# wolfbox/snappy

Hardware: AMD Instinct MI355X
Metric: GiB/s hashed (whole node), bit-exact hashes.yaml, 10k x 1 MiB tree (higher is better)
Workload: dtype u64; 1 GPU; C2: ONE on-disk tree (tmpfs) of 10001 files (10 000 x 1 MiB + the 1 MiB archive stand-in) -> hashes.yaml, sharded over 1 rank(s) on 1 distinct GPU(s); bytes=10486808576, kernel=sha512_split_kernel<true>, tree_home=/dev/shm

## Files before the change

snappy_amd/csrc/hostpass.cpp:

```cpp
#include "hostpass.h"

#include "hostfill.h"
#include "walk.h"

#include <dirent.h>
#include <errno.h>
#include <string.h>
#include <sys/stat.h>

#include <algorithm>
#include <string_view>
#include <functional>
#include <queue>
#include <thread>

namespace snaphash {


int mode_string(uint32_t st_mode, char out[11])
{
    memcpy(out, "----------", 11);
    if (S_ISDIR(st_mode)) out[0] = 'd';
    else if (S_ISLNK(st_mode)) out[0] = 'l';
    else if (S_ISREG(st_mode)) out[0] = 'f';
// ... 2 lines not shown
    for (int i = 0; i < 9; ++i)
        if (st_mode & (1u << (8 - i))) out[i + 1] = rwx[i];
    return SNAPHASH_OK;
}

int mode_parse(const char* s, uint32_t* st_mode)
{
    if (!s || !s[0]) return SNAPHASH_EPARSE;
    uint32_t m;
    switch (s[0]) {
    case 'd': m = S_IFDIR; break;
    case 'f': m = S_IFREG; break;
    case 'l': m = S_IFLNK; break;
    default: return SNAPHASH_EPARSE;
    }
    static const char rwx[] = "rwxrwxrwx";
    for (int i = 0; i < 9 && s[i + 1]; ++i)
        if (s[i + 1] == rwx[i]) m |= 1u << (8 - i);
    *st_mode = m;
    return SNAPHASH_OK;
}


static int records_from_entries_impl(std::vector<WalkEntry>& ents, std::vector<Record>& out, bool steal)
{
    if (ents.empty()) return SNAPHASH_OK;
    const size_t rootlen = ents[0].path.size();
    const size_t n = ents.size();
    const unsigned T = (unsigned)std::max<size_t>(1, std::min<size_t>(std::min(8u, usable_cpus()), n / 2048));
    std::vector<uint8_t> keep(n, 0);
    std::vector<size_t> kept(T + 1, 0), bad(T, n);
    auto range = [&](unsigned t, size_t& lo, size_t& hi) { lo = n * t / T; hi = n * (t + 1) / T; };
    run_on_threads(T, [&](unsigned t) {
        size_t lo, hi, c = 0;
        range(t, lo, hi);
        for (size_t i = lo; i < hi; ++i) {
            const char* rel = ents[i].path.c_str() + rootlen;
            if (rel[0] == 0 || strncmp(rel, "/DEBIAN", 7) == 0) continue;
            char m[11];
            if (mode_string(ents[i].st.st_mode, m) != SNAPHASH_OK) { bad[t] = i; break; }
            keep[i] = 1;
            ++c;
        }
        kept[t + 1] = c;
    });
    size_t first_bad = n;
    for (unsigned t = 0; t < T; ++t) first_bad = std::min(first_bad, bad[t]);
    if (first_bad < n) return SNAPHASH_EMODE;
    for (unsigned t = 0; t < T; ++t) kept[t + 1] += kept[t];
    const size_t base = out.size();
    out.resize(base + kept[T]);
    run_on_threads(T, [&](unsigned t) {
        size_t lo, hi;
        range(t, lo, hi);
        size_t at = base + kept[t];
        for (size_t i = lo; i < hi; ++i) {
            if (!keep[i]) continue;
            WalkEntry& e = ents[i];
            Record& r = out[at++];
            r.name.assign(e.path.c_str() + rootlen + 1, e.path.size() - rootlen - 1);
            r.st_mode = e.st.st_mode;
            r.is_regular = S_ISREG(e.st.st_mode);
            r.size = r.is_regular ? (int64_t)e.st.st_size : 0;
            if (steal) r.path = std::move(e.path);
            else r.path = e.path;
        }
    });
    return SNAPHASH_OK;
}

size_t first_unemittable_name(const std::vector<Record>& recs)
{
    const size_t n = recs.size();
    const unsigned T = (unsigned)std::max<size_t>(1, std::min<size_t>(std::min(8u, usable_cpus()), n / 2048));
    std::vector<size_t> bad(T, n);
    run_on_threads(T, [&](unsigned t) {
        for (size_t i = n * t / T; i < n * (t + 1) / T; ++i)
            if (!name_emittable(recs[i].name)) { bad[t] = i; break; }
    });
    size_t first = n;
    for (size_t b : bad) first = std::min(first, b);
    return first;
}

int records_from_entries(const std::vector<WalkEntry>& ents, std::vector<Record>& out)
{
    return records_from_entries_impl(const_cast<std::vector<WalkEntry>&>(ents), out, false);
}

int walk_tree(const char* build_dir, std::vector<Record>& out, int* err_no)
{
    std::vector<WalkEntry> ents;
    int e = 0;
    const int wrc = walk_entries(build_dir, ents, &e, nullptr);
    if (err_no) *err_no = e;
    const int rc = records_from_entries_impl(ents, out, true);
    if (rc) return rc;
    return wrc ? SNAPHASH_EIO : SNAPHASH_OK;
}


bool plain_safe_name(const std::string& s)
{
    if (s.empty() || s.size() > 72) return false;
    bool alpha = false;
    for (unsigned char c : s) {
        const bool ok = (c >= 'a' && c <= 'z') || (c >= 'A' && c <= 'Z') || (c >= '0' && c <= '9') || c == '_' ||
                        c == '.' || c == '/' || c == '-' || c == '+';
        if (!ok) return false;
        if ((c >= 'a' && c <= 'z') || (c >= 'A' && c <= 'Z')) alpha = true;
    }
    const unsigned char c0 = s[0];
    if (c0 == '-' || c0 == '.' || c0 == '+' || (c0 >= '0' && c0 <= '9')) return false;
    if (!alpha) return false;
    static const char* const resolved[] = {"y", "Y", "yes", "Yes", "YES", "on", "On", "ON", "n", "N", "no", "No", "NO",
                                           "off", "Off", "OFF", "true", "True", "TRUE", "false", "False", "FALSE",
                                           "null", "Null", "NULL", nullptr};
    if (s.size() <= 5)
        for (int i = 0; resolved[i]; ++i)
// ... 562 lines not shown
```

snappy_amd/csrc/hostpass.h:

```cpp
#pragma once
#include <stdint.h>
#include <stdio.h>

#include <string>
#include <vector>

#include "../../include/snaphash.h"

namespace snaphash {

struct Record {
    std::string name;
    std::string path;
    uint32_t st_mode = 0;
    bool is_regular = false;
    int64_t size = 0;
    std::string sha512_hex;
};

struct ParsedRecord {
    std::string name, sha512_hex;
    int64_t size = 0;
    uint32_t st_mode = 0;
    bool has_name = false, has_size = false, has_mode = false;
};
struct ParsedHashes {
    bool has_archive = false;
    std::string archive_hex;
    std::vector<ParsedRecord> files;
};

int mode_string(uint32_t st_mode, char out[11]);
int mode_parse(const char* s, uint32_t* st_mode);
int walk_tree(const char* build_dir, std::vector<Record>& out, int* err_no);
struct WalkEntry;
int records_from_entries(const std::vector<WalkEntry>& ents, std::vector<Record>& out);
bool plain_safe_name(const std::string& s);
int yaml_append_name_scalar(const std::string& s, int column, int indent, std::string& out);
bool name_emittable(const std::string& s);
size_t first_unemittable_name(const std::vector<Record>& recs);
void hex_lower(const uint8_t d[64], char out[128]);
int emit_yaml(const std::vector<Record>& recs, const uint8_t archive_digest[64], const uint8_t* file_digests,
              std::string& out);
struct YamlSkeleton {
    std::string text;
    std::vector<size_t> hex_at;
};
int emit_yaml_skeleton(const std::vector<Record>& recs, YamlSkeleton& out, unsigned max_threads = 8 );
void yaml_fill_digests(YamlSkeleton& sk, const uint8_t archive_digest[64], const uint8_t* file_digests);
int shard_listing(const char* build_dir, uint32_t rank, uint32_t world, std::string& blob, int* err_no);
int records_from_listings(const char* build_dir, uint32_t world, const void* const* blobs, const size_t* blob_lens, std::vector<Record>& recs);
int parse_yaml(const char* text, size_t len, ParsedHashes& out);
bool digest_matches_hex(const uint8_t d[64], const std::string& hex);
int lpt_assign(const uint64_t* lens, size_t n, int nshards, int32_t* shard_of);

}
```

snappy_amd/csrc/snaphash_api.cpp:

```cpp
#include <dirent.h>
#include <errno.h>
#include <fcntl.h>
#include <hip/hip_runtime.h>
#include <string.h>
#include <sys/resource.h>
#include <sys/stat.h>
#include <unistd.h>

#include <algorithm>
#include <atomic>
#include <queue>
#include <chrono>
#include <string>
#include <thread>
#include <unordered_map>
#include <vector>

#include <dlfcn.h>
#include <rccl/rccl.h>

#include <condition_variable>
#include <functional>
#include <future>
#include <memory>
#include <mutex>

#include "engine_bufs.h"
#include "hostfill.h"
#include "hostpass.h"
#include "hostsha.h"
#include "inflate_host.h"
#include "member_hashers.h"
#include "planner.h"
#include "sha512_core.h"
#include "sha512_kernels.h"
// ... 371 lines not shown
    const unsigned T = (unsigned)std::min<size_t>(cap, std::max<size_t>(1, ops.size() / 4));
    const double t_fill0 = now_ms();
    struct FillAccount {
        DevCtx* c; const std::vector<ReadOp>& ops; unsigned T; double t0;
        ~FillAccount()
        {
            uint64_t b = 0;
            for (const ReadOp& op : ops) b += op.n;
            c->fill_bytes += b;
            c->fill_thread_s += (now_ms() - t0) * 1e-3 * T;
        }
    } account{c, ops, T, t_fill0};
    c->pool.parallel_for(ops.size(), T, [&](size_t i) {
        if (first_err.load(std::memory_order_relaxed)) return;
        const ReadOp& op = ops[i];
        const int err = do_read_op(src[op.src], op, cache);
        if (err) {
            int z = 0;
            if (first_err.compare_exchange_strong(z, err)) first_err_src.store(op.src);
        }
    });
}

int hash_sources(DevCtx* c, const std::vector<Source>& src, uint8_t* digests, uint64_t* states, int* err_no,
                 int64_t* err_src)
{
    const size_t n = src.size();
    if (err_no) *err_no = 0;
    if (err_src) *err_src = -1;
    if (n == 0) return SNAPHASH_OK;
    HIP_TRY(c, hipSetDevice(c->device));
    uint64_t job_bytes = 0;
    for (const Source& sc : src) job_bytes += sc.gpu_len;
    const unsigned nslots = job_bytes > 2 * c->staging ? 3u : 2u;
    uint64_t slot_bytes = std::min<uint64_t>(c->staging, 8u << 20);
    while (slot_bytes < c->staging && slot_bytes < job_bytes / 2 + kAlign * n) slot_bytes <<= 1;
    slot_bytes = std::min(slot_bytes, c->staging);
    for (unsigned k = 0; k < nslots; ++k) slot_bytes = std::max(slot_bytes, std::min(c->slot[k].cap(), c->staging));
    int rc = ensure_slots(c, (int)nslots, slot_bytes);
    if (rc) return rc;
    HIP_TRY(c, c->hash.ensure(n, true));

    c->fill_thread_s = 0;
    c->fill_bytes = 0;
    std::vector<uint64_t> done(n, 0);
    std::vector<uint32_t> active;
    active.reserve(n);
    for (size_t i = 0; i < n; ++i)
        if (src[i].gpu_len > 0 || src[i].len == 0) active.push_back((uint32_t)i);
    std::stable_sort(active.begin(), active.end(), [&](uint32_t a, uint32_t b) { return src[a].gpu_len > src[b].gpu_len; });
    std::atomic<int> first_err{0};
    std::atomic<int64_t> first_err_src{-1};
    std::vector<ReadOp> ops;
    const bool from_memory = src[0].mem != nullptr;
    FdCache fds(from_memory ? 0 : n, c->fd_call_budget >= 0 ? std::min(c->fd_call_budget, c->fd_budget) : c->fd_budget);
    const uint64_t seg_floor = from_memory ? kMinSegmentMem : kMinSegment;
    uint64_t S_full = slot_bytes;
    if (job_bytes + kAlign * n > slot_bytes && (slot_bytes & (slot_bytes - 1)) == 0 && slot_bytes > (32u << 20)) {
        S_full = 32u << 20;
        while (S_full < slot_bytes && (S_full < job_bytes / 24 || S_full < (seg_floor + kAlign) * std::min<uint64_t>(n, kTargetStreams))) S_full <<= 1;
    }
    const unsigned per_slot = (unsigned)(slot_bytes / S_full), nsub = nslots * per_slot;
    if (c->sub.size() < nsub) c->sub.resize(nsub);
    for (unsigned q = 0; q < nsub; ++q) {
        SubSlot& ss = c->sub[q];
        if (!ss.done) HIP_TRY(c, hipEventCreateWithFlags(&ss.done, hipEventDisableTiming));
        if (!ss.copied) HIP_TRY(c, hipEventCreateWithFlags(&ss.copied, hipEventDisableTiming));
        ss.busy = false;
    }
    const size_t n_active0 = active.size();
    const size_t new_cap = [] {
        const char* e = getenv("SNAPHASH_NEW_PER_BATCH");
        return e ? (size_t)strtoul(e, nullptr, 10) : (size_t)1024;
    }();
    const bool hold_back_on = [] { const char* e = getenv("SNAPHASH_HOLD_BACK"); return !e || atoi(e) != 0; }();
    bool held_back = false;
    const unsigned ramp_shift = [] {
        const char* e = getenv("SNAPHASH_RAMP_SHIFT");
        const unsigned long v = e ? strtoul(e, nullptr, 10) : 3ul;
        return (unsigned)std::min<unsigned long>(std::max<unsigned long>(v, 1), 8);
    }();
    unsigned ramp_first64 = 24, ramp_growth_pct = 115;
    if (const char* e = getenv("SNAPHASH_RAMP_MANY")) {
        unsigned a = 0, b = 0;
        if (sscanf(e, "%u,%u", &a, &b) == 2 && a >= 1 && a <= 64 && b >= 100 && b <= 400) { ramp_first64 = a; ramp_growth_pct = b; }
    }
    unsigned batch = 0;
    double t_wait = 0, t_plan = 0, t_read = 0, t_launch = 0;
    const double t_engine0 = now_ms();
    double t_first_copy = 0;
    size_t n_copies = 0;

    while (!active.empty()) {
        const unsigned q = batch % nsub;
        SubSlot& sl = c->sub[q];
        uint8_t* const sl_h = c->slot[q / per_slot].h_buf.data() + (uint64_t)(q % per_slot) * S_full;
        uint8_t* const sl_d = c->slot[q / per_slot].d_buf.data() + (uint64_t)(q % per_slot) * S_full;
        const double tb0 = now_ms();
        if (sl.busy) { HIP_TRY(c, hipEventSynchronize(sl.done)); sl.busy = false; }
        const double tb1 = now_ms();
        t_wait += tb1 - tb0;
        long double total_rem = 0;
        size_t n_started = 0;
        for (uint32_t id : active) { total_rem += (long double)(src[id].gpu_len - done[id]); n_started += done[id] != 0; }
        uint64_t S = S_full;
        if (job_bytes + kAlign * n > S_full) {
            if (n_active0 > 2048 && ramp_growth_pct > 100) {
                double f = (double)ramp_first64 / 64.0;
                for (unsigned k = 0; k < batch && f < 1.0; ++k) f *= (double)ramp_growth_pct / 100.0;
                if (f < 1.0) S = std::max<uint64_t>((uint64_t)((double)S_full * f) & ~(uint64_t)(kAlign - 1), std::min<uint64_t>(S_full, 1u << 20));
            } else if (batch < ramp_shift) {
                const uint64_t every = active.size() <= 2048 ? std::min<uint64_t>(S_full, (seg_floor + kAlign) * (uint64_t)active.size()) : 0;
                S = std::max<uint64_t>({(S_full >> (ramp_shift - batch)) & ~(uint64_t)(kAlign - 1), every & ~(uint64_t)(kAlign - 1), std::min<uint64_t>(S_full, 1u << 20)});
            }
            if (total_rem < 2 * (long double)S) {
                const uint64_t half = ((uint64_t)(total_rem / 2) + kAlign * active.size()) & ~(uint64_t)(kAlign - 1);
                const uint64_t least = std::max<uint64_t>(S_full >> 5, (seg_floor + kAlign) * active.size());
                if (half >= least) S = std::min(S, half);
            }
        }
        const bool cap_new = new_cap != 0 && !from_memory && n_active0 > 2048;
        const size_t n_serve = cap_new ? std::min<size_t>(kTargetStreams, n_started + std::min<size_t>(new_cap, active.size() - n_started)) : kTargetStreams;
        const uint64_t floor_q = std::max<uint64_t>(seg_floor, (S / std::max<size_t>(1, n_serve)) & ~(uint64_t)(kAlign - 1));
        const uint64_t pad = kAlign * (uint64_t)active.size();
        const uint64_t S_share = pad < S / 2 ? S - pad : S;
        HIP_TRY(c, sl.jobs.ensure(active.size()));

        ops.clear();
        size_t nj = 0;
        uint64_t used = 0;
        std::vector<uint32_t> still, skipped, floor_still;
        still.reserve(active.size());
        constexpr uint64_t kHold = 16u << 10;
        const bool hold_back = hold_back_on && !held_back && n_active0 > 2048 && total_rem <= (long double)S_share && total_rem > (long double)(8u << 20) &&
                               total_rem > (long double)(kHold + kHold / 2) * (long double)active.size();
        if (hold_back) held_back = true;
        bool full = false;
        size_t n_new = 0;
        const bool share_all = total_rem > (long double)S;
        const long double share_ratio = share_all ? (long double)S_share / total_rem : 1.0L;
        for (size_t ai = 0; ai < active.size(); ++ai) {
            const uint32_t id = active[ai];
            if (full) { skipped.insert(skipped.end(), active.begin() + (ptrdiff_t)ai, active.end()); break; }
            if (cap_new && done[id] == 0 && src[id].gpu_len != 0) {
                if (n_new >= new_cap) { skipped.push_back(id); continue; }
                ++n_new;
            }
            const uint64_t rem = src[id].gpu_len - done[id];
            uint64_t quota = share_all ? (uint64_t)((long double)rem * share_ratio) : rem;
            const bool at_floor = (quota & ~(uint64_t)(kAlign - 1)) < floor_q;
            quota = std::max(quota & ~(uint64_t)(kAlign - 1), floor_q);
            uint64_t take = rem <= quota ? rem : quota;
            if (hold_back) {
                if (rem <= kHold + kHold / 2) { skipped.push_back(id); continue; }
                take = std::min<uint64_t>(take, (rem - kHold) & ~(uint64_t)(kAlign - 1));
            }
            const uint64_t at = (used + kAlign - 1) & ~(uint64_t)(kAlign - 1);
            if (at + take > S) { full = true; skipped.push_back(id); continue; }
            const bool last = take == rem;
            const bool fin = last && src[id].gpu_len == src[id].len;
            Job j;
            j.data = (uint64_t)(uintptr_t)(sl_d + at);
            j.nbytes = take;
            j.total_prev = done[id];
            j.idx = id;
            j.flags = (done[id] == 0 ? kJobFirst : 0u) | (fin ? kJobFinal : 0u);
            sl.jobs.h[nj++] = j;
            if (take) ops.push_back(ReadOp{id, done[id], take, sl_h + at, fin && src[id].path != nullptr});
            used = at + take;
            done[id] += take;
            c->stats.blocks += padded_blocks(take, fin);
            if (!last) (at_floor ? floor_still : still).push_back(id);
        }
        still.insert(still.end(), skipped.begin(), skipped.end());
        still.insert(still.end(), floor_still.begin(), floor_still.end());
        active.swap(still);
        static const bool trace_batches = getenv("SNAPHASH_TRACE_BATCHES") != nullptr;
        if (trace_batches) {
            uint64_t mx = 0;
            for (size_t k = 0; k < nj; ++k) mx = std::max<uint64_t>(mx, sl.jobs.h[k].nbytes);
            fprintf(stderr, "snaphash engine %d: batch %u: S %llu, %zu segments, %llu bytes, largest share %llu, %zu streams left behind\n", c->index, batch,
                    (unsigned long long)S, nj, (unsigned long long)used, (unsigned long long)mx, active.size());
        }
        const double tb2 = now_ms();
        t_plan += tb2 - tb1;

        run_reads(c, src, ops, first_err, first_err_src, from_memory ? nullptr : &fds, batch == 0);
        if (first_err.load()) break;
        const double tb3 = now_ms();
        t_read += tb3 - tb2;
        if (trace_batches)
            fprintf(stderr, "snaphash engine %d: batch %u: at %.2f ms: waited %.2f, planned %.2f, filled %.2f ms (%zu streams begun, %.1f GB/s)\n", c->index, batch,
                    tb0 - t_engine0, tb1 - tb0, tb2 - tb1, tb3 - tb2, n_new, (double)used / ((tb3 - tb2) * 1e6 + 1e-9));
// ... 18 lines not shown
    const double ts0 = now_ms();
    static const bool trace_tree = getenv("SNAPHASH_TRACE_TREE") != nullptr;
    float gpu_span = 0, copy_busy = 0, copy_span = 0;
    if (trace_tree && c->ev_used > 1) {
        if (c->copy_stream) (void)hipStreamSynchronize(c->copy_stream);
        (void)hipStreamSynchronize(c->stream);
        size_t first_copy = c->ev_used, last_copy = 0, last_kernel = 0;
        for (size_t i = 0; i < c->ev_used; ++i) {
            float ms = 0;
            if (c->ev_pool[i].kind == 1) {
                if (first_copy == c->ev_used) first_copy = i;
                last_copy = i;
                if (hipEventElapsedTime(&ms, c->ev_pool[i].a, c->ev_pool[i].b) == hipSuccess) copy_busy += ms;
            } else if (c->ev_pool[i].kind == 0) last_kernel = i;
        }
        if (first_copy < c->ev_used) {
            (void)hipEventElapsedTime(&gpu_span, c->ev_pool[first_copy].a, c->ev_pool[last_kernel].b);
            (void)hipEventElapsedTime(&copy_span, c->ev_pool[first_copy].a, c->ev_pool[last_copy].b);
        }
    }
    rc = sync_ctx(c);
    if (trace_tree)
        fprintf(stderr, "snaphash engine %d: %u batches; waiting for a slot %.1f ms, planning %.1f ms, reads %.1f ms, enqueue %.1f ms, drain %.1f ms; "
                        "first copy enqueued at %.2f ms, copies busy %.2f of %.2f ms, first copy -> last kernel %.2f ms, engine %.2f ms\n",
                c->index, batch, t_wait, t_plan, t_read, t_launch, now_ms() - ts0, t_first_copy, copy_busy, copy_span, gpu_span, now_ms() - t_engine0);
    for (SubSlot& ss : c->sub) ss.busy = false;
    if (rc) return rc;
    if (first_err.load()) {
        const int64_t s = first_err_src.load();
        if (err_no) *err_no = first_err.load();
        if (err_src) *err_src = s;
        return fail(c, SNAPHASH_EIO,
                    std::string(s >= 0 && src[s].path ? src[s].path : "<buffer>") + ": " + strerror(first_err.load()));
    }
    if (digests) HIP_TRY(c, hipMemcpy(digests, c->hash.d_digests.data(), n * 64, hipMemcpyDeviceToHost));
    if (states) HIP_TRY(c, hipMemcpy(states, c->hash.d_state.data(), n * 64, hipMemcpyDeviceToHost));
    for (size_t i = 0; i < n; ++i) c->stats.bytes_hashed += src[i].gpu_len;
    c->stats.streams = n;
    if (c->owner) {
        std::lock_guard<std::mutex> lk(c->owner->calib_mu);
        const double planned = c->owner->ex.planned_gpu_ms, took = now_ms() - t_engine0;
        const bool take_fill = c->staged_calls++ > 0 && !(planned > 0 && took > 3.0 * planned);
        c->owner->calib.observe_call(!from_memory, (double)c->fill_bytes, (double)n, (double)n_copies, c->stats.h2d_ms * 1e-3, c->fill_thread_s, take_fill);
    }
    return SNAPHASH_OK;
}


bool rccl_load(snaphash_ctx* x)
{
    Rccl& r = x->rccl;
    if (r.tried) return r.ok;
    r.tried = true;
    for (const char* name : {"librccl.so.1", "librccl.so", "/opt/rocm/lib/librccl.so.1"}) {
        r.lib = dlopen(name, RTLD_NOW | RTLD_LOCAL);
        if (r.lib) break;
    }
    if (!r.lib) { r.why = "librccl.so not found"; return false; }
    r.CommInitAll = (decltype(r.CommInitAll))dlsym(r.lib, "ncclCommInitAll");
    r.CommDestroy = (decltype(r.CommDestroy))dlsym(r.lib, "ncclCommDestroy");
    r.AllGather = (decltype(r.AllGather))dlsym(r.lib, "ncclAllGather");
    r.GroupStart = (decltype(r.GroupStart))dlsym(r.lib, "ncclGroupStart");
    r.GroupEnd = (decltype(r.GroupEnd))dlsym(r.lib, "ncclGroupEnd");
    r.GetErrorString = (decltype(r.GetErrorString))dlsym(r.lib, "ncclGetErrorString");
    if (!r.CommInitAll || !r.CommDestroy || !r.AllGather || !r.GroupStart || !r.GroupEnd) {
        r.why = "librccl.so lacks a required symbol";
// ... 148 lines not shown
        t.bytes_hashed += s.bytes_hashed;
        t.blocks += s.blocks;
        t.streams += s.streams;
        t.launches += s.launches;
        if (s.launches) t.kernel_used = s.kernel_used;
        t.kernel_ms = std::max(t.kernel_ms, s.kernel_ms);
        t.h2d_ms = std::max(t.h2d_ms, s.h2d_ms);
    }
    x->ex.gpu_bytes = t.bytes_hashed;
    t.bytes_hashed += x->ex.host_bytes;
    t.streams += x->ex.host_streams;
    t.wall_ms = x->stats.wall_ms;
    x->stats = t;
}

void begin_top(snaphash_ctx* x)
{
    x->stats = snaphash_stats{};
    x->ex = snaphash_stats_ex{};
    x->ex.struct_size = sizeof(snaphash_stats_ex);
    x->ex.n_devices = (uint32_t)x->dev.size();
    x->last_error.clear();
    for (auto& d : x->dev) { begin_call(d.get()); d->t_call0 = 0; }
}

bool keep_on_device_planned(const snaphash_ctx* x, size_t nd) { return nd > 1 || (x->flags & SNAPHASH_FLAG_FORCE_GATHER); }

int hash_sources_top(snaphash_ctx* x, std::vector<Source>& src, uint8_t* digests, int32_t* status)
{
    const size_t n = src.size();
    if (status) for (size_t i = 0; i < n; ++i) status[i] = 0;
    if (n == 0) return SNAPHASH_OK;
    const size_t nd = x->dev.size();
    for (Source& s : src) s.gpu_len = s.len;
    std::vector<uint8_t> on_host(n, 0);
    unsigned plan_threads = 0;
    const double t_hash0 = now_ms();
    struct HashClock {
        snaphash_ctx* x; double t0;
        ~HashClock() { x->ex.hash_ms = now_ms() - t0; }
    } hash_clock{x, t_hash0};
    if (!x->gpu_only) {
        std::vector<uint64_t> lens(n);
        for (size_t i = 0; i < n; ++i) lens[i] = src[i].len;
        PlanResult plan = plan_streams(lens.data(), n, plan_model_of(x, src[0].path != nullptr));
        on_host.swap(plan.on_host);
// ... 37 lines not shown
        DevJob& J = job[d];
        J.sub.reserve(member[d].size());
        for (uint32_t g : member[d]) J.sub.push_back(src[g]);
        if (!keep_on_device) J.dig.resize(J.sub.size() * 64);
        J.rc = hash_sources(x->dev[d].get(), J.sub, keep_on_device ? nullptr : J.dig.data(), nullptr, &J.err_no, &J.err_src);
    };

    std::atomic<size_t> hnext{0};
    std::atomic<int> herr{0};
    std::atomic<int64_t> herr_src{-1};
    unsigned nh = hidx.empty() ? 0u : std::max(1u, std::min<unsigned>(plan_threads, (unsigned)hidx.size()));
    const bool gpu_part = !gidx.empty();
    const bool spare_cores = 2u * nh <= (x->cpus_call ? x->cpus_call : x->cpus);
    std::vector<double> hbusy(std::max(1u, nh), 0.0);
    std::stable_sort(hidx.begin(), hidx.end(), [&](uint32_t a, uint32_t b) { return src[a].len > src[b].len; });
    uint64_t host_bytes_planned = 0;
    for (uint32_t g : hidx) host_bytes_planned += src[g].len;
    const uint64_t alone_from = nh ? host_bytes_planned / nh / 4 : 0;
    size_t n_lane_streams = 0;
    for (uint32_t g : hidx) n_lane_streams += src[g].len < alone_from || alone_from == 0;
    unsigned host_lanes = nh ? (unsigned)std::min<size_t>(8, (n_lane_streams + nh - 1) / nh) : 1u;
    for (auto& d : x->dev) d->fd_call_budget = -1;
    if (src[0].path != nullptr) {
        struct rlimit rl;
        int64_t soft = 1024;
        if (getrlimit(RLIMIT_NOFILE, &rl) == 0) soft = rl.rlim_cur == RLIM_INFINITY ? 65536 : (int64_t)rl.rlim_cur;
        const int64_t held = soft < 8192 ? open_descriptors() + 16 : 0;
        const int64_t reserve = std::max<int64_t>(held, std::min<int64_t>(512, soft / 2));
        const int64_t transient = gpu_part ? (int64_t)std::min(x->d0()->fill_cap, 12u) * (int64_t)nd : 0;
        const int64_t pool = std::max<int64_t>(2, soft - reserve - transient);
        int64_t lanes_fds = (int64_t)nh * host_lanes;
        const int64_t lanes_cap = gpu_part ? std::max<int64_t>(1, pool / 2) : pool;
        if (lanes_fds > lanes_cap) {
            if ((int64_t)nh > lanes_cap) nh = (unsigned)lanes_cap;
            host_lanes = (unsigned)std::max<int64_t>(1, lanes_cap / nh);
            lanes_fds = (int64_t)nh * host_lanes;
        }
        for (auto& d : x->dev) d->fd_call_budget = std::max<int64_t>(0, (pool - lanes_fds) / (int64_t)nd);
    }
    auto run_host = [&](unsigned t) {
        const double t0 = now_ms();
        int64_t bad = -1;
        const int err = host_sha512_many(
            host_lanes,
            [&]() -> int64_t {
                if (herr.load()) return -1;
                const size_t k = hnext.fetch_add(1);
                return k < hidx.size() ? (int64_t)hidx[k] : -1;
            },
            [&](int64_t g) {
                HostStream h;
                h.mem = src[g].mem;
                h.path = src[g].mem ? nullptr : src[g].path;
// ... 118 lines not shown
        ThreadJoiner th;
        for (unsigned t = 1; t < T; ++t) th.spawn(work, t);
        work(0);
        th.join_all();
        int64_t first = -1;
        for (unsigned t = 0; t < T; ++t) if (bad[t] >= 0 && (first < 0 || bad[t] < first)) first = bad[t];
        if (first >= 0) {
            int err = EIO;
            int64_t b = first_bad_path(paths, (size_t)first + 1, &err);
            if (b < 0) b = first;
            if (status) { for (size_t k = 0; k < n; ++k) status[k] = 0; status[b] = err; }
            return fail(x, SNAPHASH_EIO, std::string(paths[b]) + ": " + strerror(err));
        }
    }
    const int rc = hash_sources_top(x, src, digests, status);
    if (rc == SNAPHASH_EIO) {
        int err = 0;
        const int64_t bad = first_bad_path(paths, n, &err);
        if (bad >= 0) {
            if (status) { for (size_t k = 0; k < n; ++k) status[k] = 0; status[bad] = err; }
            return fail(x, SNAPHASH_EIO, std::string(paths[bad]) + ": " + strerror(err));
        }
    }
    return rc;
}

void end_top(snaphash_ctx* x, double t0) { x->stats.wall_ms = now_ms() - t0; }

}


extern "C" {

int snaphash_abi_version(void) { return SNAPHASH_ABI_VERSION; }

static thread_local std::string g_init_error;

static int init_fail(int code, const std::string& what, hipError_t e = hipSuccess)
try {
    g_init_error = what + (e != hipSuccess ? std::string(": ") + hipGetErrorString(e) : std::string());
    return code;
} catch (...) {
    return SNAPHASH_ENOMEM;
}

static void destroy_dev(DevCtx* c)
// ... 284 lines not shown
    c->stats.streams = n;
    return lift(x, c, launch_jobs(c, c->hash.jobs.h.data(), c->hash.jobs.d.data(), n, (uint8_t*)d_digests));
} catch (...) {
    return SNAPHASH_ENOMEM;
}

int snaphash_sync(snaphash_ctx* x)
try {
    if (!x) return SNAPHASH_EINVAL;
    for (auto& d : x->dev) {
        HIP_TRY(d.get(), hipSetDevice(d->device));
        int rc = sync_ctx(d.get());
        if (rc) return lift(x, d.get(), rc);
    }
    const double wall = x->d0()->stats.wall_ms;
    merge_stats(x);
    if (x->stats.wall_ms == 0) x->stats.wall_ms = wall;
    return SNAPHASH_OK;
} catch (...) {
    return SNAPHASH_ENOMEM;
}


static int tree_impl(snaphash_ctx* x, const char* build_dir, const char* data_tar, const uint8_t* archive_digest,
                     std::string& yaml)
{
    struct stat st;
    if (data_tar && stat(data_tar, &st) != 0) return fail(x, SNAPHASH_EIO, std::string(data_tar) + ": " + strerror(errno));
    std::vector<Record> recs;
    int en = 0;
    const double tw0 = now_ms();
    int rc = walk_tree(build_dir, recs, &en);
    const double tw1 = now_ms();
    if (rc) return fail(x, rc, rc == SNAPHASH_EIO ? std::string(build_dir) + ": " + strerror(en) : "Unknown file mode");
    if (const size_t b = first_unemittable_name(recs); b < recs.size())
        return fail(x, SNAPHASH_ENAME, "name outside what the YAML emitter restates (yamlscalar.cpp): " + recs[b].name);
    std::vector<const char*> paths;
    std::vector<int64_t> sizes;
    if (data_tar) { paths.push_back(data_tar); sizes.push_back(-1); }
    for (const Record& r : recs)
        if (r.is_regular) { paths.push_back(r.path.c_str()); sizes.push_back(r.size); }
    std::vector<uint8_t> dig(paths.size() * 64 + 64);
    const double th0 = now_ms();
    const bool early_yaml = recs.size() >= 2048;
    YamlSkeleton sk;
    int sk_rc = SNAPHASH_OK;
    ThreadJoiner skt;
    if (early_yaml) skt.spawn([&recs, &sk, &sk_rc] { sk_rc = emit_yaml_skeleton(recs, sk, 1); });
    rc = hash_paths(x, paths.data(), paths.size(), sizes.data(), dig.data(), nullptr);
    skt.join_all();
    const double th1 = now_ms();
// ... 1338 lines not shown
```

snappy_amd/csrc/walk.cpp:

```cpp
#include "walk.h"

#include "hostfill.h"

#include <dirent.h>
#include <errno.h>
#include <fcntl.h>
#include <string.h>

#include <stdio.h>
#include <stdlib.h>

#include <algorithm>
#include <atomic>
#include <chrono>
#include <thread>

namespace snaphash {

namespace {

struct Child {
    std::string name;
    unsigned char type = DT_UNKNOWN;
    struct stat st;
// ... 59 lines not shown
        const unsigned T = walk_threads(hi - lo, 4);
        std::atomic<size_t> next{lo};
        run_on_threads(T, [&](unsigned) {
            for (;;) {
                const size_t i = next.fetch_add(1);
                if (i >= hi) return;
                list_dir(dirs[i]);
            }
        });
        for (size_t i = lo; i < hi; ++i)
            for (size_t k = 0; k < dirs[i].kids.size(); ++k)
                if (dirs[i].kids[k].type == DT_DIR && !dirs[i].kids[k].lstat_errno) {
                    dirs[i].kids[k].dir = (int64_t)dirs.size();
                    DirList sub;
                    sub.path = dirs[i].path + "/" + dirs[i].kids[k].name;
                    dirs.push_back(std::move(sub));
                }
        lo = hi;
    }
}

}

int walk_entries(const char* root_c, std::vector<WalkEntry>& ents, int* err_no, std::string* err_path)
{
    std::string root(root_c);
    while (root.size() > 1 && root.back() == '/') root.pop_back();
    if (err_no) *err_no = 0;
    ents.clear();
    ents.resize(1);
    ents[0].path = root;
    if (lstat(root.c_str(), &ents[0].st) != 0) {
        if (err_no) *err_no = errno;
        if (err_path) *err_path = root;
        ents.clear();
        return -1;
    }
    ents[0].have_st = true;
    if (!S_ISDIR(ents[0].st.st_mode)) return 0;
    const bool trace = getenv("SNAPHASH_TRACE_TREE") != nullptr;
    const auto t0 = std::chrono::steady_clock::now();
    std::vector<DirList> dirs;
    list_tree(root, dirs);
    const auto t1 = std::chrono::steady_clock::now();

    const size_t nd = dirs.size();
    std::vector<size_t> count(nd, 0), start(nd, 0);
    for (size_t d = nd; d-- > 0;) {
        if (dirs[d].open_failed) { count[d] = 1; continue; }
        size_t c = 0;
        for (const Child& k : dirs[d].kids) c += 1 + (k.dir >= 0 ? count[(size_t)k.dir] : 0);
        count[d] = c;
    }
    start[0] = 1;
    struct Task { uint32_t dir, k0, k1; size_t first; };
    std::vector<Task> tasks;
    for (size_t d = 0; d < nd; ++d) {
        if (dirs[d].open_failed) { tasks.push_back(Task{(uint32_t)d, 0, 0, start[d]}); continue; }
        size_t at = start[d];
        const std::vector<Child>& kids = dirs[d].kids;
        for (size_t k = 0; k < kids.size(); ++k) {
            if (k % 256 == 0) tasks.push_back(Task{(uint32_t)d, (uint32_t)k, (uint32_t)std::min(kids.size(), k + 256), at});
            if (kids[k].dir >= 0) { start[(size_t)kids[k].dir] = at + 1; at += 1 + count[(size_t)kids[k].dir]; }
            else at += 1;
        }
    }
    const size_t n = 1 + count[0];
    ents.resize(n);

    const unsigned T = walk_threads(n, 512);
    std::vector<int64_t> bad(T, -1);
    std::vector<int> bad_errno(T, 0);
    std::atomic<size_t> next{0};
    auto work = [&](unsigned t) {
        auto fail = [&](size_t idx, int e) { if (bad[t] < 0 || (int64_t)idx < bad[t]) { bad[t] = (int64_t)idx; bad_errno[t] = e; } };
        for (;;) {
            const size_t ti = next.fetch_add(1);
            if (ti >= tasks.size()) return;
            const Task& tk = tasks[ti];
            const DirList& dl = dirs[tk.dir];
            if (dl.open_failed) {
                WalkEntry& e = ents[tk.first];
                e.path = dl.path;
                if (lstat(e.path.c_str(), &e.st) != 0) fail(tk.first, errno);
                else e.have_st = true;
                continue;
            }
            size_t at = tk.first;
            for (uint32_t k = tk.k0; k < tk.k1; ++k) {
                const Child& c = dl.kids[k];
                WalkEntry& e = ents[at];
                e.path.reserve(dl.path.size() + 1 + c.name.size());
                e.path = dl.path;
                e.path += '/';
                e.path += c.name;
                if (c.lstat_errno) fail(at, c.lstat_errno);
                else if (c.have_st) { e.st = c.st; e.have_st = true; }
                else if ((dl.kept ? fstatat(dirfd(dl.kept), c.name.c_str(), &e.st, AT_SYMLINK_NOFOLLOW) : lstat(e.path.c_str(), &e.st)) != 0) fail(at, errno);
                else e.have_st = true;
                at += 1 + (c.dir >= 0 ? count[(size_t)c.dir] : 0);
            }
        }
    };
    struct ReleaseDirs {
        std::vector<DirList>& dirs;
        ~ReleaseDirs()
        {
            int n = 0;
            for (DirList& d : dirs) if (d.kept) { d.release(); ++n; }
            g_kept_dirs.fetch_sub(n);
        }
    } release_dirs{dirs};
    run_on_threads(T, work);
    if (trace) {
        const auto t2 = std::chrono::steady_clock::now();
        fprintf(stderr, "snaphash walk: listing %zu directories (readdir + sort) %.2f ms, paths + Lstat of %zu entries on %u threads %.2f ms\n", nd,
                std::chrono::duration<double, std::milli>(t1 - t0).count(), n, T, std::chrono::duration<double, std::milli>(t2 - t1).count());
    }
    int64_t first_bad = -1;
    int first_errno = 0;
    for (unsigned t = 0; t < T; ++t)
        if (bad[t] >= 0 && (first_bad < 0 || bad[t] < first_bad)) { first_bad = bad[t]; first_errno = bad_errno[t]; }
    if (first_bad < 0) return 0;
    if (err_no) *err_no = first_errno;
// ... 7 lines not shown
```

snappy_amd/csrc/walk.h:

```cpp
#pragma once
#include <sys/stat.h>

#include <string>
#include <vector>

namespace snaphash {

struct WalkEntry {
    std::string path;
    struct stat st;
    bool have_st = false;
};

int walk_entries(const char* root, std::vector<WalkEntry>& ents, int* err_no, std::string* err_path);

}
```

Before: 50.44 GiB/s.

## Stream walked files into the GPU hash engine while the tree walk continues

Adds a streaming path for the single-GPU tree case. The walker pushes stat'd regular files into a shared feed, and the hash engine starts copying and hashing once about 1024 files are listed, instead of waiting for the full walk and record build. Batch sizing uses an estimate of the total bytes while the feed is open, and the tail-halving and hold-back heuristics are turned off during streaming. This overlaps walk latency with H2D and kernel work, but it adds mutex and condition-variable traffic, changes the ramp parameters, and depends on byte estimates that can misjudge slot sizing.

```diff
diff --git a/snappy_amd/csrc/hostpass.cpp b/snappy_amd/csrc/hostpass.cpp
--- a/snappy_amd/csrc/hostpass.cpp
+++ b/snappy_amd/csrc/hostpass.cpp
@@ -48,7 +48,8 @@
 }
 
 
-static int records_from_entries_impl(std::vector<WalkEntry>& ents, std::vector<Record>& out, bool steal)
+static int records_from_entries_impl(std::vector<WalkEntry>& ents, std::vector<Record>& out, bool steal,
+                                     std::vector<size_t>* entry_of = nullptr)
 {
     if (ents.empty()) return SNAPHASH_OK;
     const size_t rootlen = ents[0].path.size();
@@ -76,12 +77,14 @@
     for (unsigned t = 0; t < T; ++t) kept[t + 1] += kept[t];
     const size_t base = out.size();
     out.resize(base + kept[T]);
+    if (entry_of) entry_of->resize(base + kept[T]);
     run_on_threads(T, [&](unsigned t) {
         size_t lo, hi;
         range(t, lo, hi);
         size_t at = base + kept[t];
         for (size_t i = lo; i < hi; ++i) {
             if (!keep[i]) continue;
+            if (entry_of) (*entry_of)[at] = i;
             WalkEntry& e = ents[i];
             Record& r = out[at++];
             r.name.assign(e.path.c_str() + rootlen + 1, e.path.size() - rootlen - 1);
@@ -116,11 +119,16 @@
 
 int walk_tree(const char* build_dir, std::vector<Record>& out, int* err_no)
 {
+    return walk_tree(build_dir, out, err_no, nullptr, nullptr);
+}
+
+int walk_tree(const char* build_dir, std::vector<Record>& out, int* err_no, const WalkSink* sink, std::vector<size_t>* entry_of)
+{
     std::vector<WalkEntry> ents;
     int e = 0;
-    const int wrc = walk_entries(build_dir, ents, &e, nullptr);
+    const int wrc = walk_entries(build_dir, ents, &e, nullptr, sink);
     if (err_no) *err_no = e;
-    const int rc = records_from_entries_impl(ents, out, true);
+    const int rc = records_from_entries_impl(ents, out, true, entry_of);
     if (rc) return rc;
     return wrc ? SNAPHASH_EIO : SNAPHASH_OK;
 }
diff --git a/snappy_amd/csrc/hostpass.h b/snappy_amd/csrc/hostpass.h
--- a/snappy_amd/csrc/hostpass.h
+++ b/snappy_amd/csrc/hostpass.h
@@ -34,6 +34,8 @@
 int mode_parse(const char* s, uint32_t* st_mode);
 int walk_tree(const char* build_dir, std::vector<Record>& out, int* err_no);
 struct WalkEntry;
+struct WalkSink;
+int walk_tree(const char* build_dir, std::vector<Record>& out, int* err_no, const WalkSink* sink, std::vector<size_t>* entry_of);
 int records_from_entries(const std::vector<WalkEntry>& ents, std::vector<Record>& out);
 bool plain_safe_name(const std::string& s);
 int yaml_append_name_scalar(const std::string& s, int column, int indent, std::string& out);
diff --git a/snappy_amd/csrc/snaphash_api.cpp b/snappy_amd/csrc/snaphash_api.cpp
--- a/snappy_amd/csrc/snaphash_api.cpp
+++ b/snappy_amd/csrc/snaphash_api.cpp
@@ -11,6 +11,7 @@
 #include <atomic>
 #include <queue>
 #include <chrono>
+#include <deque>
 #include <string>
 #include <thread>
 #include <unordered_map>
@@ -428,16 +429,53 @@
     });
 }
 
-int hash_sources(DevCtx* c, const std::vector<Source>& src, uint8_t* digests, uint64_t* states, int* err_no,
-                 int64_t* err_src)
-{
-    const size_t n = src.size();
+struct Feed {
+    std::mutex mu;
+    std::condition_variable cv;
+    std::deque<std::string> paths;
+    std::vector<Source> pending;
+    std::vector<size_t> entry;
+    size_t n_max = 0;
+    size_t entries = 0, entries_done = 0;
+    uint64_t bytes = 0;
+    bool listed = false;
+    bool finished = false;
+    bool failed = false;
+    std::vector<uint8_t> digests;
+};
+
+int hash_sources(DevCtx* c, std::vector<Source>& src, uint8_t* digests, uint64_t* states, int* err_no,
+                 int64_t* err_src, Feed* feed = nullptr)
+{
     if (err_no) *err_no = 0;
     if (err_src) *err_src = -1;
-    if (n == 0) return SNAPHASH_OK;
+    bool feed_open = false, feed_failed = false;
+    size_t n_expect = 0;
+    uint64_t job_est = 0;
+    const double t_feed0 = now_ms();
+    auto take_feed = [&](std::unique_lock<std::mutex>&) {
+        const size_t first = src.size();
+        src.insert(src.end(), feed->pending.begin(), feed->pending.end());
+        feed->pending.clear();
+        feed_open = !feed->finished;
+        feed_failed = feed->failed;
+        if (feed_open) job_est = std::max<uint64_t>(feed->bytes, feed->entries_done ? (uint64_t)((long double)feed->bytes * feed->entries / feed->entries_done) : 0);
+        return first;
+    };
+    if (feed) {
+        std::unique_lock<std::mutex> lk(feed->mu);
+        feed->cv.wait(lk, [&] { return feed->finished || (feed->listed && feed->entry.size() >= 1024); });
+        take_feed(lk);
+        n_expect = feed->n_max;
+        if (feed_failed) return SNAPHASH_OK;
+    }
+    const double t_feed_wait = now_ms() - t_feed0;
+    const size_t n = feed_open ? n_expect : src.size();
+    if (src.empty()) return SNAPHASH_OK;
     HIP_TRY(c, hipSetDevice(c->device));
-    uint64_t job_bytes = 0;
-    for (const Source& sc : src) job_bytes += sc.gpu_len;
+    uint64_t job_bytes = feed_open ? job_est : 0;
+    for (const Source& sc : src) job_bytes += feed_open ? 0 : sc.gpu_len;
+    uint64_t assigned = 0;
     const unsigned nslots = job_bytes > 2 * c->staging ? 3u : 2u;
     uint64_t slot_bytes = std::min<uint64_t>(c->staging, 8u << 20);
     while (slot_bytes < c->staging && slot_bytes < job_bytes / 2 + kAlign * n) slot_bytes <<= 1;
@@ -452,9 +490,13 @@
     std::vector<uint64_t> done(n, 0);
     std::vector<uint32_t> active;
     active.reserve(n);
-    for (size_t i = 0; i < n; ++i)
-        if (src[i].gpu_len > 0 || src[i].len == 0) active.push_back((uint32_t)i);
-    std::stable_sort(active.begin(), active.end(), [&](uint32_t a, uint32_t b) { return src[a].gpu_len > src[b].gpu_len; });
+    auto enlist = [&](size_t from) {
+        const size_t a0 = active.size();
+        for (size_t i = from; i < src.size(); ++i)
+            if (src[i].gpu_len > 0 || src[i].len == 0) active.push_back((uint32_t)i);
+        std::stable_sort(active.begin() + (ptrdiff_t)a0, active.end(), [&](uint32_t a, uint32_t b) { return src[a].gpu_len > src[b].gpu_len; });
+    };
+    enlist(0);
     std::atomic<int> first_err{0};
     std::atomic<int64_t> first_err_src{-1};
     std::vector<ReadOp> ops;
@@ -474,7 +516,7 @@
         if (!ss.copied) HIP_TRY(c, hipEventCreateWithFlags(&ss.copied, hipEventDisableTiming));
         ss.busy = false;
     }
-    const size_t n_active0 = active.size();
+    const size_t n_active0 = feed_open ? n_expect : active.size();
     const size_t new_cap = [] {
         const char* e = getenv("SNAPHASH_NEW_PER_BATCH");
         return e ? (size_t)strtoul(e, nullptr, 10) : (size_t)1024;
@@ -486,7 +528,7 @@
         const unsigned long v = e ? strtoul(e, nullptr, 10) : 3ul;
         return (unsigned)std::min<unsigned long>(std::max<unsigned long>(v, 1), 8);
     }();
-    unsigned ramp_first64 = 24, ramp_growth_pct = 115;
+    unsigned ramp_first64 = feed ? 32 : 24, ramp_growth_pct = feed ? 110 : 115;
     if (const char* e = getenv("SNAPHASH_RAMP_MANY")) {
         unsigned a = 0, b = 0;
         if (sscanf(e, "%u,%u", &a, &b) == 2 && a >= 1 && a <= 64 && b >= 100 && b <= 400) { ramp_first64 = a; ramp_growth_pct = b; }
@@ -497,7 +539,14 @@
     double t_first_copy = 0;
     size_t n_copies = 0;
 
-    while (!active.empty()) {
+    for (;;) {
+        if (feed_open) {
+            std::unique_lock<std::mutex> lk(feed->mu);
+            if (active.empty()) feed->cv.wait(lk, [&] { return feed->finished || !feed->pending.empty(); });
+            enlist(take_feed(lk));
+            if (feed_failed) break;
+        }
+        if (active.empty()) break;
         const unsigned q = batch % nsub;
         SubSlot& sl = c->sub[q];
         uint8_t* const sl_h = c->slot[q / per_slot].h_buf.data() + (uint64_t)(q % per_slot) * S_full;
@@ -519,7 +568,7 @@
                 const uint64_t every = active.size() <= 2048 ? std::min<uint64_t>(S_full, (seg_floor + kAlign) * (uint64_t)active.size()) : 0;
                 S = std::max<uint64_t>({(S_full >> (ramp_shift - batch)) & ~(uint64_t)(kAlign - 1), every & ~(uint64_t)(kAlign - 1), std::min<uint64_t>(S_full, 1u << 20)});
             }
-            if (total_rem < 2 * (long double)S) {
+            if (!feed_open && total_rem < 2 * (long double)S) {
                 const uint64_t half = ((uint64_t)(total_rem / 2) + kAlign * active.size()) & ~(uint64_t)(kAlign - 1);
                 const uint64_t least = std::max<uint64_t>(S_full >> 5, (seg_floor + kAlign) * active.size());
                 if (half >= least) S = std::min(S, half);
@@ -538,13 +587,14 @@
         std::vector<uint32_t> still, skipped, floor_still;
         still.reserve(active.size());
         constexpr uint64_t kHold = 16u << 10;
-        const bool hold_back = hold_back_on && !held_back && n_active0 > 2048 && total_rem <= (long double)S_share && total_rem > (long double)(8u << 20) &&
+        const bool hold_back = hold_back_on && !held_back && !feed_open && n_active0 > 2048 && total_rem <= (long double)S_share && total_rem > (long double)(8u << 20) &&
                                total_rem > (long double)(kHold + kHold / 2) * (long double)active.size();
         if (hold_back) held_back = true;
         bool full = false;
         size_t n_new = 0;
-        const bool share_all = total_rem > (long double)S;
-        const long double share_ratio = share_all ? (long double)S_share / total_rem : 1.0L;
+        const long double share_of = feed_open ? std::max(total_rem, (long double)(job_est > assigned ? job_est - assigned : 0)) : total_rem;
+        const bool share_all = share_of > (long double)S;
+        const long double share_ratio = share_all ? (long double)S_share / share_of : 1.0L;
         for (size_t ai = 0; ai < active.size(); ++ai) {
             const uint32_t id = active[ai];
             if (full) { skipped.insert(skipped.end(), active.begin() + (ptrdiff_t)ai, active.end()); break; }
@@ -575,6 +625,7 @@
             if (take) ops.push_back(ReadOp{id, done[id], take, sl_h + at, fin && src[id].path != nullptr});
             used = at + take;
             done[id] += take;
+            assigned += take;
             c->stats.blocks += padded_blocks(take, fin);
             if (!last) (at_floor ? floor_still : still).push_back(id);
         }
@@ -639,10 +690,12 @@
     rc = sync_ctx(c);
     if (trace_tree)
         fprintf(stderr, "snaphash engine %d: %u batches; waiting for a slot %.1f ms, planning %.1f ms, reads %.1f ms, enqueue %.1f ms, drain %.1f ms; "
-                        "first copy enqueued at %.2f ms, copies busy %.2f of %.2f ms, first copy -> last kernel %.2f ms, engine %.2f ms\n",
-                c->index, batch, t_wait, t_plan, t_read, t_launch, now_ms() - ts0, t_first_copy, copy_busy, copy_span, gpu_span, now_ms() - t_engine0);
+                        "first copy enqueued at %.2f ms, copies busy %.2f of %.2f ms, first copy -> last kernel %.2f ms, engine %.2f ms%s\n",
+                c->index, batch, t_wait, t_plan, t_read, t_launch, now_ms() - ts0, t_first_copy, copy_busy, copy_span, gpu_span, now_ms() - t_engine0,
+                feed ? (" (after " + std::to_string(t_feed_wait) + " ms waiting for the walk's first files)").c_str() : "");
     for (SubSlot& ss : c->sub) ss.busy = false;
     if (rc) return rc;
+    if (feed_failed) return SNAPHASH_OK;
     if (first_err.load()) {
         const int64_t s = first_err_src.load();
         if (err_no) *err_no = first_err.load();
@@ -650,15 +703,19 @@
         return fail(c, SNAPHASH_EIO,
                     std::string(s >= 0 && src[s].path ? src[s].path : "<buffer>") + ": " + strerror(first_err.load()));
     }
-    if (digests) HIP_TRY(c, hipMemcpy(digests, c->hash.d_digests.data(), n * 64, hipMemcpyDeviceToHost));
-    if (states) HIP_TRY(c, hipMemcpy(states, c->hash.d_state.data(), n * 64, hipMemcpyDeviceToHost));
-    for (size_t i = 0; i < n; ++i) c->stats.bytes_hashed += src[i].gpu_len;
-    c->stats.streams = n;
+    if (feed) {
+        feed->digests.resize(src.size() * 64);
+        digests = feed->digests.data();
+    }
+    if (digests) HIP_TRY(c, hipMemcpy(digests, c->hash.d_digests.data(), src.size() * 64, hipMemcpyDeviceToHost));
+    if (states) HIP_TRY(c, hipMemcpy(states, c->hash.d_state.data(), src.size() * 64, hipMemcpyDeviceToHost));
+    for (const Source& sc : src) c->stats.bytes_hashed += sc.gpu_len;
+    c->stats.streams = src.size();
     if (c->owner) {
         std::lock_guard<std::mutex> lk(c->owner->calib_mu);
         const double planned = c->owner->ex.planned_gpu_ms, took = now_ms() - t_engine0;
         const bool take_fill = c->staged_calls++ > 0 && !(planned > 0 && took > 3.0 * planned);
-        c->owner->calib.observe_call(!from_memory, (double)c->fill_bytes, (double)n, (double)n_copies, c->stats.h2d_ms * 1e-3, c->fill_thread_s, take_fill);
+        c->owner->calib.observe_call(!from_memory, (double)c->fill_bytes, (double)src.size(), (double)n_copies, c->stats.h2d_ms * 1e-3, c->fill_thread_s, take_fill);
     }
     return SNAPHASH_OK;
 }
@@ -853,6 +910,17 @@
     x->ex.n_devices = (uint32_t)x->dev.size();
     x->last_error.clear();
     for (auto& d : x->dev) { begin_call(d.get()); d->t_call0 = 0; }
+}
+
+int64_t descriptor_pool(const snaphash_ctx* x, bool gpu_part)
+{
+    struct rlimit rl;
+    int64_t soft = 1024;
+    if (getrlimit(RLIMIT_NOFILE, &rl) == 0) soft = rl.rlim_cur == RLIM_INFINITY ? 65536 : (int64_t)rl.rlim_cur;
+    const int64_t held = soft < 8192 ? open_descriptors() + 16 : 0;
+    const int64_t reserve = std::max<int64_t>(held, std::min<int64_t>(512, soft / 2));
+    const int64_t transient = gpu_part ? (int64_t)std::min(x->d0()->fill_cap, 12u) * (int64_t)x->dev.size() : 0;
+    return std::max<int64_t>(2, soft - reserve - transient);
 }
 
 bool keep_on_device_planned(const snaphash_ctx* x, size_t nd) { return nd > 1 || (x->flags & SNAPHASH_FLAG_FORCE_GATHER); }
@@ -936,13 +1004,7 @@
     unsigned host_lanes = nh ? (unsigned)std::min<size_t>(8, (n_lane_streams + nh - 1) / nh) : 1u;
     for (auto& d : x->dev) d->fd_call_budget = -1;
     if (src[0].path != nullptr) {
-        struct rlimit rl;
-        int64_t soft = 1024;
-        if (getrlimit(RLIMIT_NOFILE, &rl) == 0) soft = rl.rlim_cur == RLIM_INFINITY ? 65536 : (int64_t)rl.rlim_cur;
-        const int64_t held = soft < 8192 ? open_descriptors() + 16 : 0;
-        const int64_t reserve = std::max<int64_t>(held, std::min<int64_t>(512, soft / 2));
-        const int64_t transient = gpu_part ? (int64_t)std::min(x->d0()->fill_cap, 12u) * (int64_t)nd : 0;
-        const int64_t pool = std::max<int64_t>(2, soft - reserve - transient);
+        const int64_t pool = descriptor_pool(x, gpu_part);
         int64_t lanes_fds = (int64_t)nh * host_lanes;
         const int64_t lanes_cap = gpu_part ? std::max<int64_t>(1, pool / 2) : pool;
         if (lanes_fds > lanes_cap) {
@@ -1107,6 +1169,24 @@
             return fail(x, SNAPHASH_EIO, std::string(paths[bad]) + ": " + strerror(err));
         }
     }
+    return rc;
+}
+
+int hash_feed_top(snaphash_ctx* x, Feed& feed)
+{
+    const double t_hash0 = now_ms();
+    struct HashClock {
+        snaphash_ctx* x; double t0;
+        ~HashClock() { x->ex.hash_ms = now_ms() - t0; x->ex.gpu_ms = x->ex.hash_ms; }
+    } hash_clock{x, t_hash0};
+    DevCtx* c = x->d0();
+    c->fd_call_budget = descriptor_pool(x, true);
+    std::vector<Source> src;
+    int err_no = 0;
+    int64_t err_src = -1;
+    const int rc = hash_sources(c, src, nullptr, nullptr, &err_no, &err_src, &feed);
+    if (rc) x->last_error = c->last_error;
+    merge_stats(x);
     return rc;
 }
 
@@ -1437,11 +1517,126 @@
 }
 
 
+static int tree_streamed(snaphash_ctx* x, const char* build_dir, const char* data_tar, const struct stat& tar_st,
+                         const uint8_t* archive_digest, std::string& yaml)
+{
+    Feed feed;
+    if (data_tar) {
+        feed.paths.emplace_back(data_tar);
+        Source sc;
+        sc.path = feed.paths.back().c_str();
+        sc.len = sc.gpu_len = (uint64_t)tar_st.st_size;
+        feed.pending.push_back(sc);
+        feed.entry.push_back(SIZE_MAX);
+        feed.bytes = sc.len;
+    }
+    WalkSink sink;
+    sink.listed = [&feed](size_t n) {
+        { std::lock_guard<std::mutex> lk(feed.mu); feed.entries = n; feed.n_max = feed.entry.size() + n; feed.listed = true; }
+        feed.cv.notify_one();
+    };
+    sink.chunk = [&feed](std::vector<WalkFile>& files, size_t entries) {
+        {
+            std::lock_guard<std::mutex> lk(feed.mu);
+            for (WalkFile& f : files) {
+                feed.paths.push_back(std::move(f.path));
+                Source sc;
+                sc.path = feed.paths.back().c_str();
+                sc.len = sc.gpu_len = (uint64_t)f.size;
+                feed.pending.push_back(sc);
+                feed.entry.push_back(f.entry);
+                feed.bytes += sc.len;
+            }
+            feed.entries_done += entries;
+        }
+        if (!files.empty()) feed.cv.notify_one();
+    };
+    std::vector<Record> recs;
+    std::vector<size_t> entry_of;
+    int walk_rc = SNAPHASH_OK, en = 0;
+    std::string walk_msg;
+    std::exception_ptr walk_threw;
+    bool early_yaml = false;
+    YamlSkeleton sk;
+    int sk_rc = SNAPHASH_OK;
+    const double tw0 = now_ms();
+    double tw1 = tw0;
+    auto walker = [&] {
+        try {
+            walk_rc = walk_tree(build_dir, recs, &en, &sink, &entry_of);
+            if (walk_rc) walk_msg = walk_rc == SNAPHASH_EIO ? std::string(build_dir) + ": " + strerror(en) : "Unknown file mode";
+            else if (const size_t b = first_unemittable_name(recs); b < recs.size()) {
+                walk_rc = SNAPHASH_ENAME;
+                walk_msg = "name outside what the YAML emitter restates (yamlscalar.cpp): " + recs[b].name;
+            }
+        } catch (...) {
+            walk_threw = std::current_exception();
+        }
+        tw1 = now_ms();
+        { std::lock_guard<std::mutex> lk(feed.mu); feed.finished = true; feed.failed = walk_rc != SNAPHASH_OK || walk_threw; }
+        feed.cv.notify_one();
+        if (!walk_rc && !walk_threw && recs.size() >= 2048) {
+            early_yaml = true;
+            sk_rc = emit_yaml_skeleton(recs, sk, 1);
+        }
+    };
+    int rc;
+    {
+        ThreadJoiner wt;
+        wt.spawn(walker);
+        rc = hash_feed_top(x, feed);
+        wt.join_all();
+    }
+    const double th1 = now_ms();
+    if (walk_threw) std::rethrow_exception(walk_threw);
+    if (walk_rc) return fail(x, walk_rc, walk_msg);
+    const size_t base = data_tar ? 1 : 0;
+    std::vector<int64_t> row_of(feed.entries, -1);
+    size_t rows = base;
+    for (size_t k = 0; k < recs.size(); ++k)
+        if (recs[k].is_regular) row_of[entry_of[k]] = (int64_t)rows++;
+    if (rc == SNAPHASH_EIO) {
+        std::vector<const char*> paths;
+        if (data_tar) paths.push_back(data_tar);
+        for (const Record& r : recs)
+            if (r.is_regular) paths.push_back(r.path.c_str());
+        int err = 0;
+        const int64_t bad = first_bad_path(paths.data(), paths.size(), &err);
+        if (bad >= 0) return fail(x, SNAPHASH_EIO, std::string(paths[bad]) + ": " + strerror(err));
+    }
+    if (rc) return rc;
+    std::vector<uint8_t> dig(rows * 64 + 64);
+    size_t placed = 0;
+    for (size_t k = 0; k < feed.entry.size(); ++k) {
+        const int64_t r = feed.entry[k] == SIZE_MAX ? 0 : row_of[feed.entry[k]];
+        if (r < 0) continue;
+        memcpy(dig.data() + 64 * (size_t)r, feed.digests.data() + 64 * k, 64);
+        ++placed;
+    }
+    if (placed != rows) return fail(x, SNAPHASH_EIO, std::string(build_dir) + ": the tree changed while it was walked");
+    const uint8_t* arch = data_tar ? dig.data() : archive_digest;
+    const uint8_t* files = data_tar ? dig.data() + 64 : dig.data();
+    if (early_yaml) {
+        rc = sk_rc;
+        if (!rc) { yaml_fill_digests(sk, arch, files); yaml.swap(sk.text); }
+    } else {
+        rc = emit_yaml(recs, arch, files, yaml);
+    }
+    static const bool trace_tree = getenv("SNAPHASH_TRACE_TREE") != nullptr;
+    if (trace_tree)
+        fprintf(stderr, "snaphash tree (walk streamed): walk %.1f ms (%zu records), walk + hash %.1f ms (%zu streams), yaml %.1f ms (%zu bytes)\n",
+                tw1 - tw0, recs.size(), th1 - tw0, feed.entry.size(), now_ms() - th1, yaml.size());
+    return rc;
+}
+
 static int tree_impl(snaphash_ctx* x, const char* build_dir, const char* data_tar, const uint8_t* archive_digest,
                      std::string& yaml)
 {
     struct stat st;
     if (data_tar && stat(data_tar, &st) != 0) return fail(x, SNAPHASH_EIO, std::string(data_tar) + ": " + strerror(errno));
+    const bool stream_walk = [] { const char* e = getenv("SNAPHASH_STREAM_WALK"); return !e || atoi(e) != 0; }();
+    if (stream_walk && x->gpu_only && x->dev.size() == 1 && !(x->flags & SNAPHASH_FLAG_FORCE_GATHER) && !(data_tar && S_ISDIR(st.st_mode)))
+        return tree_streamed(x, build_dir, data_tar, st, archive_digest, yaml);
     std::vector<Record> recs;
     int en = 0;
     const double tw0 = now_ms();
diff --git a/snappy_amd/csrc/walk.cpp b/snappy_amd/csrc/walk.cpp
--- a/snappy_amd/csrc/walk.cpp
+++ b/snappy_amd/csrc/walk.cpp
@@ -105,7 +105,12 @@
 
 }
 
-int walk_entries(const char* root_c, std::vector<WalkEntry>& ents, int* err_no, std::string* err_path)
+int walk_entries(const char* root, std::vector<WalkEntry>& ents, int* err_no, std::string* err_path)
+{
+    return walk_entries(root, ents, err_no, err_path, nullptr);
+}
+
+int walk_entries(const char* root_c, std::vector<WalkEntry>& ents, int* err_no, std::string* err_path, const WalkSink* sink)
 {
     std::string root(root_c);
     while (root.size() > 1 && root.back() == '/') root.pop_back();
@@ -120,7 +125,15 @@
         return -1;
     }
     ents[0].have_st = true;
-    if (!S_ISDIR(ents[0].st.st_mode)) return 0;
+    if (!S_ISDIR(ents[0].st.st_mode)) {
+        if (sink) {
+            sink->listed(1);
+            std::vector<WalkFile> one;
+            if (S_ISREG(ents[0].st.st_mode)) one.push_back(WalkFile{0, ents[0].path, (int64_t)ents[0].st.st_size});
+            sink->chunk(one, 1);
+        }
+        return 0;
+    }
     const bool trace = getenv("SNAPHASH_TRACE_TREE") != nullptr;
     const auto t0 = std::chrono::steady_clock::now();
     std::vector<DirList> dirs;
@@ -150,6 +163,11 @@
     }
     const size_t n = 1 + count[0];
     ents.resize(n);
+    if (sink) {
+        sink->listed(n);
+        std::vector<WalkFile> none;
+        sink->chunk(none, 1);
+    }
 
     const unsigned T = walk_threads(n, 512);
     std::vector<int64_t> bad(T, -1);
@@ -167,8 +185,15 @@
                 e.path = dl.path;
                 if (lstat(e.path.c_str(), &e.st) != 0) fail(tk.first, errno);
                 else e.have_st = true;
+                if (sink) {
+                    std::vector<WalkFile> again;
+                    if (e.have_st && S_ISREG(e.st.st_mode)) again.push_back(WalkFile{tk.first, e.path, (int64_t)e.st.st_size});
+                    sink->chunk(again, e.have_st ? 1 : 0);
+                }
                 continue;
             }
+            std::vector<WalkFile> files;
+            size_t stated = 0;
             size_t at = tk.first;
             for (uint32_t k = tk.k0; k < tk.k1; ++k) {
                 const Child& c = dl.kids[k];
@@ -181,8 +206,13 @@
                 else if (c.have_st) { e.st = c.st; e.have_st = true; }
                 else if ((dl.kept ? fstatat(dirfd(dl.kept), c.name.c_str(), &e.st, AT_SYMLINK_NOFOLLOW) : lstat(e.path.c_str(), &e.st)) != 0) fail(at, errno);
                 else e.have_st = true;
+                if (sink && e.have_st) {
+                    ++stated;
+                    if (S_ISREG(e.st.st_mode)) files.push_back(WalkFile{at, e.path, (int64_t)e.st.st_size});
+                }
                 at += 1 + (c.dir >= 0 ? count[(size_t)c.dir] : 0);
             }
+            if (sink) sink->chunk(files, stated);
         }
     };
     struct ReleaseDirs {
diff --git a/snappy_amd/csrc/walk.h b/snappy_amd/csrc/walk.h
--- a/snappy_amd/csrc/walk.h
+++ b/snappy_amd/csrc/walk.h
@@ -1,6 +1,7 @@
 #pragma once
 #include <sys/stat.h>
 
+#include <functional>
 #include <string>
 #include <vector>
 
@@ -14,4 +15,17 @@
 
 int walk_entries(const char* root, std::vector<WalkEntry>& ents, int* err_no, std::string* err_path);
 
+struct WalkFile {
+    size_t entry;
+    std::string path;
+    int64_t size;
+};
+
+struct WalkSink {
+    std::function<void(size_t)> listed;
+    std::function<void(std::vector<WalkFile>&, size_t)> chunk;
+};
+
+int walk_entries(const char* root, std::vector<WalkEntry>& ents, int* err_no, std::string* err_path, const WalkSink* sink);
+
 }
```

After: 50.95 GiB/s, median of 6. +1.0%, better.
